# samedii/perceptor

Measured on AMD Instinct MI355X. Metric: denoising steps/sec (UNet+CLIP-grad) at 512x512 batch 8, higher is better.
Workload: dtype bf16

## Files before the change

perceptor_amd/csrc/gemm_wd.hip:

```cpp
#include "common.h"
#include "../../include/perceptor_hip.h"

namespace {

template <typename T, int MB, bool TWO = false, int NWV = 8, bool CONV = false>
__global__ __launch_bounds__(NWV * 64, 2) void gemm_wd_kernel(const pmi_igemm_args a) {
  constexpr int TM = 16 * MB, BN = NWV * 32, BK = 128, NT = NWV * 64;
  constexpr int ROW = 2 * BK + 32;
  constexpr int TILE = TM * ROW;
  constexpr int NPI = (TM * 16 + NT - 1) / NT;
  constexpr int HIMG = TM * (BN * 2 + 16);
  __shared__ __attribute__((aligned(16))) char smem[2 * TILE > 2 * HIMG ? 2 * TILE : 2 * HIMG];

  const int tid = threadIdx.x, lane = tid & 63;
  const int wid = __builtin_amdgcn_readfirstlane(tid >> 6);
#ifdef PMI_STAMPS
#define GSTAMP(k) do { if (tid == 0 && a.reserved == 77 && a.splitk <= 1) ((long long*)a.ws)[(int64_t)blockIdx.x * 8 + (k)] = (long long)wall_clock64(); } while (0)
#else
#define GSTAMP(k) do {} while (0)
#endif
  GSTAMP(0);
  const int tiles_n = (a.N + BN - 1) / BN, tiles_m = (a.M + TM - 1) / TM;
  const int logical = xcd_remap(blockIdx.x, tiles_m * tiles_n);
  const bool mfast = (int64_t)a.M <= (int64_t)a.N;
// ... 249 lines not shown
      }
      float v[4] = {c[0] * a.alpha + bv.x, c[1] * a.alpha + bv.y, c[2] * a.alpha + bv.z, c[3] * a.alpha + bv.w};
#pragma unroll
      for (int e = 0; e < 4; ++e) v[e] = act_apply(v[e], ACT);
      if (a.R) {
        if (a.res_f32) {
          const float4 rr = *(const float4*)((const float*)a.R + (int64_t)m * a.ldr + n);
          v[0] += rr.x; v[1] += rr.y; v[2] += rr.z; v[3] += rr.w;
        } else {
          const uint2 rr = *(const uint2*)((const u16*)a.R + (int64_t)m * a.ldr + n);
          v[0] += T::to_f((u16)(rr.x & 0xffff)); v[1] += T::to_f((u16)(rr.x >> 16));
          v[2] += T::to_f((u16)(rr.y & 0xffff)); v[3] += T::to_f((u16)(rr.y >> 16));
        }
      }
      if (a.out_f32) *(float4*)((float*)a.D + (int64_t)m * a.ldd + n) = make_float4(v[0], v[1], v[2], v[3]);
      else *(uint2*)((u16*)a.D + (int64_t)m * a.ldd + n) = pack4<T>(v[0], v[1], v[2], v[3]);
    }
  }
  });
  GSTAMP(3);
}

static int g_few_wgs = 128;

template <typename T>
int launch(const pmi_igemm_args& a, hipStream_t s, int mb) {
  const int tm = 16 * mb;
  const bool few = a.splitk <= 1 && (long)((a.M + 127) / 128) * ((a.N + 255) / 256) < g_few_wgs && !a.D2 && !a.aux && a.act != PMI_ACT_GEGLU;
  const bool half_tail = (a.N % 256) != 0 && (a.N % 256) <= 128 && a.N < 1024;
  if (a.N < 256 || few || half_tail) {
    const dim3 g4(((a.M + 127) / 128) * ((a.N + 127) / 128), 1, a.splitk > 1 ? a.splitk : 1);
    if (a.taps == 9) {
      if (a.A1) hipLaunchKernelGGL((gemm_wd_kernel<T, 8, true, 4, true>), g4, dim3(256), 0, s, a);
      else hipLaunchKernelGGL((gemm_wd_kernel<T, 8, false, 4, true>), g4, dim3(256), 0, s, a);
    } else if (a.A1) hipLaunchKernelGGL((gemm_wd_kernel<T, 8, true, 4>), g4, dim3(256), 0, s, a);
    else hipLaunchKernelGGL((gemm_wd_kernel<T, 8, false, 4>), g4, dim3(256), 0, s, a);
    PMI_CHECK_LAUNCH();
    return PMI_OK;
  }
  const dim3 grid(((a.M + tm - 1) / tm) * ((a.N + 255) / 256), 1, a.splitk > 1 ? a.splitk : 1);
  if (a.taps == 9) {
    if (a.A1) hipLaunchKernelGGL((gemm_wd_kernel<T, 8, true, 8, true>), grid, dim3(512), 0, s, a);
    else hipLaunchKernelGGL((gemm_wd_kernel<T, 8, false, 8, true>), grid, dim3(512), 0, s, a);
  } else if (a.A1) hipLaunchKernelGGL((gemm_wd_kernel<T, 8, true>), grid, dim3(512), 0, s, a);
  else if (mb == 9) hipLaunchKernelGGL((gemm_wd_kernel<T, 9>), grid, dim3(512), 0, s, a);
  else hipLaunchKernelGGL((gemm_wd_kernel<T, 8>), grid, dim3(512), 0, s, a);
  PMI_CHECK_LAUNCH();
  return PMI_OK;
}

}

void pmi_gemm_wd_few_wgs(int v) { g_few_wgs = v; }

int pmi_gemm_wd_tile_rows(const pmi_igemm_args* a, int splitk) {
  if (a->A1 || a->taps == 9 || a->N < 256 || ((a->N % 256) != 0 && (a->N % 256) <= 128 && a->N < 1024)) return 128;
  if (splitk <= 1 && (long)((a->M + 127) / 128) * ((a->N + 255) / 256) < g_few_wgs && !a->D2 && !a->aux && a->act != PMI_ACT_GEGLU) return 128;
  int best = 8;
  long best_cost = -1;
  for (int mb = 8; mb <= 9; ++mb) {
    const long wgs = (long)((a->M + 16 * mb - 1) / (16 * mb)) * ((a->N + 255) / 256) * (splitk > 1 ? splitk : 1);
    const long cost = ((wgs + 255) / 256) * mb;
    if (best_cost < 0 || cost < best_cost) { best_cost = cost; best = mb; }
  }
  return 16 * best;
}

int pmi_igemm_halo_allowed(void);

extern "C" int pmi_gemm_wd_eligible(const pmi_igemm_args* a) {
  if (!a->Bf || (a->taps != 1 && a->taps != 9) || a->up || a->stride != 1 || a->batch > 1) return 0;
  if (a->taps == 9) {
    if ((a->C0 % 128) || (a->A1 ? (a->C1 <= 0 || (a->C1 % 128)) : a->C1 != 0) || a->D2 || a->aux || a->act == PMI_ACT_GEGLU || a->split_in) return 0;
    if (a->H <= 0 || a->W <= 0 || a->H >= 0x4000 || a->W >= 0x4000 || a->Hin != a->H || a->Win != a->W || (a->M % (a->H * a->W))) return 0;
    if (a->K != 9 * (a->C0 + a->C1) || (int64_t)a->M * (a->lda0 > a->lda1 ? a->lda0 : a->lda1) * 2 >= ((int64_t)1 << 31)) return 0;
    if (pmi_igemm_halo_allowed() && pmi_conv3x3_halo_config(a) >= 0) return 0;
    if (a->M < 512) return 0;
  } else {
    if (a->A1 ? (a->C1 <= 0 || (a->C0 % 128) || (a->C1 % 32) || a->splitk > 1 || a->D2 || a->aux || a->act == PMI_ACT_GEGLU) : a->C1 != 0) return 0;
    if (a->K != a->C0 + a->C1) return 0;
  }
  if (a->nbias && (a->taps != 9 || a->splitk == 1)) return 0;
  if (a->res_up && (a->taps != 9 || a->splitk == 1)) return 0;
  if (a->stats || a->pro_a || a->split_out) return 0;
  if ((a->K % 32) || (a->N % 32) || a->M < 64) return 0;
  if (a->N < 256 && a->N != 128) return 0;
  if ((a->N % 256) && a->N < 1024) {
    const int tail = a->N % 256;
    if (tail < 64) return 0;
  }
  if ((a->D2 || a->aux) && (a->out_f32 || a->splitk > 1 || (a->R && a->res_f32))) return 0;
  if (a->act == PMI_ACT_GEGLU && (a->R || a->D2 || a->aux || a->out_f32 || a->splitk > 1)) return 0;
  return 1;
}

int pmi_gemm_wd_launch(const pmi_igemm_args* a, void* stream) {
  hipStream_t s = (hipStream_t)stream;
  const int mb = pmi_gemm_wd_tile_rows(a, a->splitk) / 16;
  return a->dtype == PMI_DT_BF16 ? launch<BF16>(*a, s, mb) : launch<F16>(*a, s, mb);
}
```

perceptor_amd/csrc/igemm.hip:

```cpp
#include <cstdio>
#include <cstdlib>
#include "common.h"
#include "epilogue.h"
#include "../../include/perceptor_hip.h"

namespace {

constexpr int BM = 128, BN = 128, BK = 64;
constexpr int TILE_BYTES = 128 * 128;
constexpr int STAGE_BYTES = 2 * TILE_BYTES;

__device__ __forceinline__ int lds_off(int row, int chunk) { return row * 128 + ((chunk ^ ((row >> 1) & 7)) << 4); }

template <typename T, bool CONV, bool KFAST, bool PHASED = false>
__global__ __launch_bounds__(256, 2) void igemm_kernel(const pmi_igemm_args a) {
  static_assert(!PHASED || CONV, "the phased geometry is a convolution");
  __shared__ __attribute__((aligned(16))) char smem[2 * STAGE_BYTES];

  const int tid = threadIdx.x, lane = tid & 63, wid = tid >> 6;
  const int wr = wid >> 1, wc = wid & 1;
#ifdef PMI_STAMPS
#define GSTAMP(k) do { if (tid == 0 && a.reserved == 77 && a.splitk <= 1) ((long long*)a.ws)[(int64_t)blockIdx.x * 8 + (k)] = (long long)wall_clock64(); } while (0)
#else
#define GSTAMP(k) do {} while (0)
// ... 338 lines not shown
    if (a.R) {
#pragma unroll
      for (int i = 0; i < 2; ++i)
#pragma unroll
        for (int g = 0; g < 4; ++g) {
          const int n = n0 + wc * 64 + j * 32 + 4 * lhi + 8 * g;
          rv[i][g] = make_float4(0.f, 0.f, 0.f, 0.f);
          if (mrow[i] >= a.M || n >= a.N) continue;
          if (a.res_f32) {
            rv[i][g] = *(const float4*)((const float*)a.R + offR + rrow[i] + n);
          } else if (a.split_out) {
            const int po = split_off(n, a.split_out);
            const uint2 rh = *(const uint2*)((const u16*)a.R + offR + rrow[i] + po);
            const uint2 rl = *(const uint2*)((const u16*)a.R + offR + rrow[i] + po + a.split_out);
            rv[i][g].x = __builtin_bit_cast(float, rh.x); rv[i][g].y = __builtin_bit_cast(float, rh.y);
            rv[i][g].z = __builtin_bit_cast(float, rl.x); rv[i][g].w = __builtin_bit_cast(float, rl.y);
          } else {
            const uint2 r = *(const uint2*)((const u16*)a.R + offR + rrow[i] + n);
            rv[i][g].x = __builtin_bit_cast(float, r.x); rv[i][g].y = __builtin_bit_cast(float, r.y);
          }
        }
    }
#pragma unroll
    for (int i = 0; i < 2; ++i) {
      const int m = mrow[i];
      if (m >= Mr) continue;
      const int64_t mo = orow(m);
#pragma unroll
      for (int g = 0; g < 4; ++g) {
        const int n = n0 + wc * 64 + j * 32 + 4 * lhi + 8 * g;
        if (n >= a.N) continue;
        float v[4];
#pragma unroll
        for (int e = 0; e < 4; ++e) v[e] = acc[i][j][4 * g + e] * a.alpha;
        v[0] += bv[g].x + nbv[i][g].x; v[1] += bv[g].y + nbv[i][g].y; v[2] += bv[g].z + nbv[i][g].z; v[3] += bv[g].w + nbv[i][g].w;
        if (a.act != PMI_ACT_NONE) act_apply_n<4>(v, a.act);
        if (a.R) {
          if (a.res_f32) {
            v[0] += rv[i][g].x; v[1] += rv[i][g].y; v[2] += rv[i][g].z; v[3] += rv[i][g].w;
          } else {
            const uint32_t r0 = __builtin_bit_cast(uint32_t, rv[i][g].x), r1 = __builtin_bit_cast(uint32_t, rv[i][g].y);
            v[0] += T::to_f((u16)(r0 & 0xffff)); v[1] += T::to_f((u16)(r0 >> 16));
            v[2] += T::to_f((u16)(r1 & 0xffff)); v[3] += T::to_f((u16)(r1 >> 16));
            if (a.split_out) {
              const uint32_t l0 = __builtin_bit_cast(uint32_t, rv[i][g].z), l1 = __builtin_bit_cast(uint32_t, rv[i][g].w);
              v[0] += T::to_f((u16)(l0 & 0xffff)); v[1] += T::to_f((u16)(l0 >> 16));
              v[2] += T::to_f((u16)(l1 & 0xffff)); v[3] += T::to_f((u16)(l1 >> 16));
            }
          }
        }
        if (a.split_out) {
          const int64_t o = offD + (int64_t)m * a.ldd + split_off(n, a.split_out);
          const uint2 hi = pack4<T>(v[0], v[1], v[2], v[3]);
          const float l0 = v[0] - T::to_f((u16)(hi.x & 0xffff)), l1 = v[1] - T::to_f((u16)(hi.x >> 16));
          const float l2 = v[2] - T::to_f((u16)(hi.y & 0xffff)), l3 = v[3] - T::to_f((u16)(hi.y >> 16));
          *(uint2*)((u16*)a.D + o) = hi;
          *(uint2*)((u16*)a.D + o + a.split_out) = pack4<T>(l0, l1, l2, l3);
        } else {
        const int64_t o = offD + mo * a.ldd + n;
        if (a.out_f32) *(float4*)((float*)a.D + o) = make_float4(v[0], v[1], v[2], v[3]);
        else *(uint2*)((u16*)a.D + o) = pack4<T>(v[0], v[1], v[2], v[3]);
        }
#pragma unroll
        for (int e = 0; e < 4; ++e) { ssum[4 * g + e] += v[e]; ssq[4 * g + e] += v[e] * v[e]; }
      }
    }
    if (a.stats) stats_block_to_lds(ssum, ssq, stat + wr * 2 * BN, wc * 64 + j * 32, lane);
  }
  }
  if (a.stats) {
    __syncthreads();
    const int img = m0 / a.hw, prow = (m0 - img * a.hw) / BM;
    float* o = a.stats + ((int64_t)(img * a.stats_p + prow) * a.N + n0) * 2;
    for (int c = tid; c < 2 * BN; c += 256)
      if (n0 + (c >> 1) < a.N) o[c] = stat[c] + stat[2 * BN + c];
  }
#ifdef PMI_STAMPS
  __syncthreads();
  GSTAMP(3);
#endif
}

template <typename T>
__global__ __launch_bounds__(256) void splitk_reduce_kernel(const pmi_igemm_args a) {
  const int n4 = a.N >> 2;
  const int64_t total = (int64_t)a.M * n4;
  const float* ws = (const float*)a.ws;
  for (int64_t i = (int64_t)blockIdx.x * 256 + threadIdx.x; i < total; i += (int64_t)gridDim.x * 256) {
    const int m = (int)(i / n4), n = (int)(i - (int64_t)m * n4) * 4;
    float4 s = make_float4(0.f, 0.f, 0.f, 0.f);
    for (int z = 0; z < a.splitk; ++z) {
      const float4 p = *(const float4*)(ws + ((int64_t)z * a.M + m) * a.N + n);
      s.x += p.x; s.y += p.y; s.z += p.z; s.w += p.w;
    }
    float v[4] = {s.x * a.alpha, s.y * a.alpha, s.z * a.alpha, s.w * a.alpha};
    if (a.bias) { const float4 b = *(const float4*)(a.bias + n); v[0] += b.x; v[1] += b.y; v[2] += b.z; v[3] += b.w; }
    if (a.nbias) {
      const float4 b = *(const float4*)(a.nbias + (int64_t)(m / a.hw) * (a.ldnb ? a.ldnb : a.N) + n);
      v[0] += b.x; v[1] += b.y; v[2] += b.z; v[3] += b.w;
    }
    if (a.act != PMI_ACT_NONE) act_apply_n<4>(v, a.act);
    if (a.R) {
      int64_t rrow = (int64_t)m * a.ldr;
      if (a.res_up) {
        const int hw = a.H * a.W;
        const int img = m / hw, rem = m - img * hw;
        const int y = rem / a.W, x = rem - y * a.W;
        rrow = ((int64_t)(img * (a.H >> 1) + (y >> 1)) * (a.W >> 1) + (x >> 1)) * a.ldr;
      }
      if (a.res_f32) {
        const float4 r = *(const float4*)((const float*)a.R + rrow + n);
        v[0] += r.x; v[1] += r.y; v[2] += r.z; v[3] += r.w;
      } else {
        const int po = a.split_out ? split_off(n, a.split_out) : n;
        const uint2 r = *(const uint2*)((const u16*)a.R + rrow + po);
        v[0] += T::to_f((u16)(r.x & 0xffff)); v[1] += T::to_f((u16)(r.x >> 16));
        v[2] += T::to_f((u16)(r.y & 0xffff)); v[3] += T::to_f((u16)(r.y >> 16));
        if (a.split_out) {
          const uint2 l = *(const uint2*)((const u16*)a.R + rrow + po + a.split_out);
          v[0] += T::to_f((u16)(l.x & 0xffff)); v[1] += T::to_f((u16)(l.x >> 16));
          v[2] += T::to_f((u16)(l.y & 0xffff)); v[3] += T::to_f((u16)(l.y >> 16));
        }
      }
    }
    if (a.split_out) {
      const int64_t o = (int64_t)m * a.ldd + split_off(n, a.split_out);
      const uint2 hi = pack4<T>(v[0], v[1], v[2], v[3]);
      const float l0 = v[0] - T::to_f((u16)(hi.x & 0xffff)), l1 = v[1] - T::to_f((u16)(hi.x >> 16));
      const float l2 = v[2] - T::to_f((u16)(hi.y & 0xffff)), l3 = v[3] - T::to_f((u16)(hi.y >> 16));
      *(uint2*)((u16*)a.D + o) = hi;
      *(uint2*)((u16*)a.D + o + a.split_out) = pack4<T>(l0, l1, l2, l3);
      continue;
    }
    const int64_t o = (int64_t)m * a.ldd + n;
    if (a.out_f32) *(float4*)((float*)a.D + o) = make_float4(v[0], v[1], v[2], v[3]);
    else *(uint2*)((u16*)a.D + o) = pack4<T>(v[0], v[1], v[2], v[3]);
  }
}

template <typename T>
int launch(const pmi_igemm_args& a, hipStream_t s) {
  const bool phased = a.up == 2;
  const int tiles = (((phased ? a.M / 4 : a.M) + BM - 1) / BM) * ((a.N + BN - 1) / BN);
  const dim3 grid(tiles, phased ? 4 : 1, a.batch > 1 ? a.batch : (a.splitk > 1 ? a.splitk : 1)), block(256);
  const bool conv = a.taps != 1 || a.up || a.stride == 2;
  const int Cin = a.C0 + a.C1;
  const bool kfast = (Cin % BK == 0) && (a.C0 % BK == 0);
  if (phased) {
    if (kfast) hipLaunchKernelGGL((igemm_kernel<T, true, true, true>), grid, block, 0, s, a);
    else hipLaunchKernelGGL((igemm_kernel<T, true, false, true>), grid, block, 0, s, a);
  } else if (conv) {
    if (kfast) hipLaunchKernelGGL((igemm_kernel<T, true, true>), grid, block, 0, s, a);
    else hipLaunchKernelGGL((igemm_kernel<T, true, false>), grid, block, 0, s, a);
  } else {
    if (kfast) hipLaunchKernelGGL((igemm_kernel<T, false, true>), grid, block, 0, s, a);
    else hipLaunchKernelGGL((igemm_kernel<T, false, false>), grid, block, 0, s, a);
  }
  PMI_CHECK_LAUNCH();
  if (a.splitk > 1) {
    const int64_t work = (int64_t)a.M * (a.N / 4);
    const int blocks = (int)((work + 255) / 256 > 4096 ? 4096 : (work + 255) / 256);
    hipLaunchKernelGGL(splitk_reduce_kernel<T>, dim3(blocks), dim3(256), 0, s, a);
    PMI_CHECK_LAUNCH();
  }
  return PMI_OK;
}

}

extern "C" int pmi_conv3x3_halo_config(const pmi_igemm_args* a);
int pmi_conv3x3_halo_launch(const pmi_igemm_args* a, int cfg, void* stream);
int pmi_conv3x3_wd_launch(const pmi_igemm_args* a, int cfg, void* stream);
extern "C" int pmi_gemm_wd_eligible(const pmi_igemm_args* a);
int pmi_gemm_wd_tile_rows(const pmi_igemm_args* a, int splitk);
int pmi_gemm_wd_launch(const pmi_igemm_args* a, void* stream);
void pmi_conv3x3_allow_wd(int v);
void pmi_conv3x3_wd_mf16(int v);
void pmi_conv3x3_wd128(int v);
void pmi_conv3x3_force_config(int cfg);
void pmi_conv3x3_prefer_256(int v);
static int g_allow_halo = 1;
static int g_wd_max_split = 8;
int pmi_conv3x3_wd_splitk(const pmi_igemm_args* a, int cfg);
extern "C" int pmi_igemm_splitk(const pmi_igemm_args* a) {
  if (a->batch > 1 || (a->N & 3) || a->up == 2) return 1;
  if (g_allow_halo) {
    const int halo = pmi_conv3x3_halo_config(a);
    if (halo >= 0) return pmi_conv3x3_wd_splitk(a, halo);
  }
  if (a->act == PMI_ACT_GEGLU) return 1;
  if (a->A1 && a->taps == 1 && pmi_gemm_wd_eligible(a)) return 1;
  if (pmi_gemm_wd_eligible(a)) {
    const int nch = (a->K + 127) / 128;
    int best = 1;
    long best_cost = -1;
    for (int s = 1; s <= g_wd_max_split && nch / s >= 4; s *= 2) {
      const int rows = pmi_gemm_wd_tile_rows(a, s);
      const long wgs = (long)((a->M + rows - 1) / rows) * (a->N < 256 ? 1 : (a->N + 255) / 256) * s;
      const long cost = ((wgs + 255) / 256) * rows * (nch / s + 6) + (s > 1 ? 8L * 144 : 0);
      if (best_cost < 0 || cost < best_cost) { best_cost = cost; best = s; }
    }
    return best;
  }
  const int tiles = ((a->M + BM - 1) / BM) * ((a->N + BN - 1) / BN);
  const int nk = (a->K + BK - 1) / BK;
  if (tiles >= 384 || nk < 16) return 1;
  int s = 512 / tiles;
  if (s > nk / 8) s = nk / 8;
  if (s > 16) s = 16;
  return s < 2 ? 1 : s;
}

int pmi_igemm_halo_allowed(void) { return g_allow_halo; }

extern "C" int pmi_igemm_stats_rows(const pmi_igemm_args* a) {
  if (a->batch > 1 || a->splitk > 1 || a->up == 2) return 0;
  const int halo = g_allow_halo ? pmi_conv3x3_halo_config(a) : -1;
  if (a->split_out) return halo >= 6 ? (a->H / 8) * (a->W / 32) : 0;
  if (halo == 3) return 0;
  if (halo >= 0) return (a->H / (halo == 1 ? 16 : 8)) * (a->W / 32);
  if (a->hw > 0 && (a->hw % BM) == 0 && (a->M % a->hw) == 0) return a->hw / BM;
  return 0;
}

void pmi_attn_flash_qt(int v);
void pmi_attn_flash_kv_chunks(int v);
void pmi_conv3x3_wd_splitk_enable(int v);
void pmi_gemm_wd_few_wgs(int v);
void pmi_conv3x3_wd_smallc(int v);

extern "C" int pmi_set_option(int key, int value) {
  if (key == 0) { const int old = g_allow_halo; g_allow_halo = value; return old; }
  if (key == 1) { pmi_conv3x3_force_config(value); return 0; }
  if (key == 2) { pmi_conv3x3_prefer_256(value); return 0; }
  if (key == 6) { pmi_conv3x3_allow_wd(value); return 0; }
  if (key == 7) { pmi_conv3x3_wd_mf16(value); return 0; }
  if (key == 8) { pmi_conv3x3_wd128(value); return 0; }
  if (key == 9) { pmi_attn_flash_qt(value); return 0; }
  if (key == 10) { pmi_conv3x3_wd_splitk_enable(value); return 0; }
  if (key == 11) { g_wd_max_split = value; return 0; }
  if (key == 12) { pmi_gemm_wd_few_wgs(value); return 0; }
  if (key == 13) { pmi_conv3x3_wd_smallc(value); return 0; }
  if (key == 14) { pmi_attn_flash_kv_chunks(value); return 0; }
  return PMI_ERR_ARG;
}

static int bad_arg(int line) {
  if (getenv("PMI_DEBUG")) fprintf(stderr, "pmi_igemm: argument check at igemm.hip:%d failed\n", line);
  return PMI_ERR_ARG;
}

extern "C" int pmi_igemm(const pmi_igemm_args* a, pmi_stream_t stream) {
  if (!a || !a->A0 || !a->B || !a->D) return bad_arg(__LINE__);
  if (a->M <= 0 || a->N <= 0 || a->K <= 0) return bad_arg(__LINE__);
  if ((a->K & 7) || (a->C0 & 7) || (a->C1 & 7)) return bad_arg(__LINE__);
  if ((a->N & 3) && (a->bias || a->nbias || a->R || a->ldd < ((a->N + 3) & ~3))) return bad_arg(__LINE__);
  if ((a->lda0 & 7) || (a->ldb & 7) || (a->ldd & 3)) return bad_arg(__LINE__);
  if (a->C1 > 0 && (!a->A1 || (a->lda1 & 7))) return bad_arg(__LINE__);
  if (a->taps != 1 && a->taps != 9 && a->taps != 16) return bad_arg(__LINE__);
  if (a->taps == 16 && (a->stride != 2 || a->up || a->res_up || a->Hin != 2 * a->H || a->Win != 2 * a->W)) return bad_arg(__LINE__);
  if (a->stride != 1 && a->stride != 2) return bad_arg(__LINE__);
  if (a->up == 2 && (a->taps != 9 || a->stride != 2 || a->res_up || a->A1 || a->C1 || a->R || a->nbias || a->stats || a->splitk > 1 || a->batch > 1 ||
                     a->split_out || a->split_in || a->pro_a || a->D2 || a->aux || a->dtype == PMI_DT_F16X2 || (a->M & 3))) return bad_arg(__LINE__);
  if (a->K != a->taps * (a->C0 + a->C1)) return bad_arg(__LINE__);
  if (a->R && (a->ldr & 3)) return bad_arg(__LINE__);
  if (a->split_out && ((a->split_out & 7) || a->split_out > 32 || a->out_f32 || (a->N % a->split_out) || a->batch > 1)) return bad_arg(__LINE__);
  if ((unsigned)a->split_in > 2u) return bad_arg(__LINE__);
  if (a->split_in == 2 && !a->split_out) return bad_arg(__LINE__);
  if (a->nbias && a->hw <= 0) return bad_arg(__LINE__);
  const bool conv = a->taps != 1 || a->up || a->stride == 2;
  if (a->res_up && ((a->H & 1) || (a->W & 1))) return bad_arg(__LINE__);
  if ((conv || a->res_up) && (a->H <= 0 || a->W <= 0 || a->Hin <= 0 || a->Win <= 0 || a->M % (a->H * a->W))) return bad_arg(__LINE__);
  if (a->up && (a->H != 2 * a->Hin || a->W != 2 * a->Win)) return bad_arg(__LINE__);
  if (a->batch > 1 && a->batch_inner <= 0) return bad_arg(__LINE__);
  const int halo = g_allow_halo ? pmi_conv3x3_halo_config(a) : -1;
  if (a->pro_a && (!a->pro_b || halo < 0)) return PMI_ERR_ARG;
  if ((a->split_in == 2 || ((a->split_in || a->split_out) && a->pro_a) || (a->split_out && a->R && a->res_f32)) && halo < 6) return bad_arg(__LINE__);
  if (a->stats && a->stats_p != pmi_igemm_stats_rows(a)) return PMI_ERR_ARG;
  if (a->splitk > 1 && (!a->ws || a->batch > 1 || (halo >= 0 && a->splitk != pmi_conv3x3_wd_splitk(a, halo)) || (a->N & 3) || a->stats)) return PMI_ERR_ARG;
  if (a->act == PMI_ACT_GEGLU && !pmi_gemm_wd_eligible(a)) return bad_arg(__LINE__);
  if ((a->D2 || a->aux) && !pmi_gemm_wd_eligible(a)) return bad_arg(__LINE__);
  if (pmi_gemm_wd_eligible(a) && !((a->nbias || a->res_up) && a->splitk <= 1)) {
    const int rc = pmi_gemm_wd_launch(a, stream);
    if (rc != PMI_OK || a->splitk <= 1 || a->reserved3 == 1) return rc;
    hipStream_t s = (hipStream_t)stream;
    const int64_t work = (int64_t)a->M * (a->N / 4);
    const int blocks = (int)((work + 255) / 256 > 4096 ? 4096 : (work + 255) / 256);
    if (a->dtype == PMI_DT_BF16) hipLaunchKernelGGL(splitk_reduce_kernel<BF16>, dim3(blocks), dim3(256), 0, s, *a);
    else hipLaunchKernelGGL(splitk_reduce_kernel<F16>, dim3(blocks), dim3(256), 0, s, *a);
    PMI_CHECK_LAUNCH();
    return PMI_OK;
  }
  if (halo >= 4) {
    const int rc = pmi_conv3x3_wd_launch(a, halo, stream);
    if (rc != PMI_OK || a->splitk <= 1) return rc;
    hipStream_t s = (hipStream_t)stream;
    const int64_t work = (int64_t)a->M * (a->N / 4);
    const int blocks = (int)((work + 255) / 256 > 4096 ? 4096 : (work + 255) / 256);
    if (a->dtype == PMI_DT_BF16) hipLaunchKernelGGL(splitk_reduce_kernel<BF16>, dim3(blocks), dim3(256), 0, s, *a);
    else hipLaunchKernelGGL(splitk_reduce_kernel<F16>, dim3(blocks), dim3(256), 0, s, *a);
    PMI_CHECK_LAUNCH();
    return PMI_OK;
  }
  if (halo >= 0) return pmi_conv3x3_halo_launch(a, halo, stream);
  hipStream_t s = (hipStream_t)stream;
  return a->dtype == PMI_DT_BF16 ? launch<BF16>(*a, s) : launch<F16>(*a, s);
}

extern "C" int pmi_abi_version(void) { return 1; }
```

perceptor_amd/engine/ops.py:

```python
from __future__ import annotations

import math
import os
import ctypes as C
from typing import Optional

import torch

from .. import _hip
from .._hip import ACT_GEGLU, ACT_NONE, DT_F16X2, IgemmArgs, call, ptr


HALO_ENABLED = True
SPLITK_ENABLED = True
WD_ENABLED = True
GEMM_WD_ENABLED = True
GEMM_WD_CONV = os.environ.get("PMI_GEMM_WD_CONV", "1") != "0"
FLASH_ENABLED = True


def set_halo(enabled: bool) -> None:
    global HALO_ENABLED
    HALO_ENABLED = bool(enabled)
    _hip.lib().pmi_set_option(0, int(enabled))
# ... 251 lines not shown
    a.pro_a, a.pro_b, a.pro_act = ptr(ca), ptr(cb), pact
    out = _empty((n, h, w, 2 * lin.n_p), torch.float16, x.device)
    a.D, a.ldd = ptr(out), out.stride(-2)
    rows = _hip.lib().pmi_igemm_stats_rows(C.byref(a))
    if rows > 0:
        st = _empty((n, rows, lin.n_p, 2), torch.float32, x.device)
        a.stats, a.stats_p = ptr(st), rows
        out._pmi_stats = (st, rows)
    if DEBUG_WS is not None:
        a.ws = ptr(DEBUG_WS)
        a.reserved = 77
    if KERNEL_EVENTS is not None:
        e0, e1 = torch.cuda.Event(enable_timing=True), torch.cuda.Event(enable_timing=True)
        e0.record()
        call("pmi_igemm", C.byref(a))
        e1.record()
        nbytes = (x.numel() + (x1.numel() if x1 is not None else 0)) * 2 + lin.w.numel() * 2 + out.numel() * 2 + (residual.numel() * 2 if residual is not None else 0)
        KERNEL_EVENTS.append((e0, e1, 2.0 * m * lin.cout * lin.cin * 9, float(nbytes), f"{h}x{w} {c0}+{c1}->{lin.cout} cfg{cfg} mixed-{operand}"))
        return out
    call("pmi_igemm", C.byref(a))
    return out


def igemm(a0: torch.Tensor, lin: PackedLinear, *, a1: Optional[torch.Tensor] = None, residual: Optional[torch.Tensor] = None,
          act: int = ACT_NONE, up: bool = False, stride: int = 1, res_up: bool = False, nbias: Optional[torch.Tensor] = None,
          out_f32: bool = False, out: Optional[torch.Tensor] = None, alpha: float = 1.0, prologue=None,
          want_stats: bool = False, hw: Optional[int] = None, pre_out: Optional[torch.Tensor] = None,
          act_grad_of: Optional[torch.Tensor] = None, act_grad: int = ACT_NONE, defer_reduce: bool = False,
          split_out: bool = False) -> torch.Tensor:
    dt = lin.dt
    conv = a0.ndim == 4
    if lin.concat_inputs and a1 is not None and prologue is None:
        a0, a1 = torch.cat([a0, a1], dim=-1), None
    c0 = a0.shape[-1]
    c1 = a1.shape[-1] if a1 is not None else 0
    assert (c0 + c1) * (2 if lin.self_concat else 1) == lin.cin_p, (c0, c1, lin.cin_p)
    a = IgemmArgs()
    if conv:
        n, hin, win, _ = a0.shape
        hv, wv = (hin * 2, win * 2) if up else (hin, win)
        h, w = hv // stride, wv // stride
        m = n * h * w
        a.H, a.W, a.Hin, a.Win = h, w, hin, win
        a.hw = h * w
        oshape = (n, h, w, lin.n_p)
    else:
        assert lin.taps == 1 and not up and stride == 1
        m = a0.shape[0]
        a.hw = hw or 1
        oshape = (m, lin.n_p // 2 if act == ACT_GEGLU else lin.n_p)
    if lin.split:
        a.split_in = 1
    if (lin.split and not out_f32) or split_out:
        a.split_out = split_group(lin.n_p)
        oshape = oshape[:-1] + (2 * lin.n_p,)
    if out is None:
        out = _empty(oshape, torch.float32 if out_f32 else _hip.TORCH_DTYPE[dt], a0.device)
    a.A0, a.A1, a.B = ptr(a0), ptr(a1), ptr(lin.w)
    a.bias, a.nbias, a.R, a.D = ptr(lin.b), ptr(nbias), ptr(residual), ptr(out)
    a.M, a.N, a.K = m, lin.n_p, lin.K
    a.C0, a.C1 = c0, c1
    a.lda0, a.lda1 = a0.stride(-2), (a1.stride(-2) if a1 is not None else 0)
    a.ldb, a.ldd = lin.K, out.stride(-2)
    a.ldr = residual.stride(-2) if residual is not None else 0
    a.taps, a.stride, a.up, a.res_up, a.act = lin.taps, stride, int(up), int(res_up), act
    a.out_f32 = int(out.dtype == torch.float32)
    a.res_f32 = int(residual is not None and residual.dtype == torch.float32)
    a.alpha = alpha
    a.ldnb = nbias.stride(0) if nbias is not None else 0
    a.batch, a.batch_inner = 1, 1
    a.dtype = dt
    if conv and lin.taps == 9 and stride == 1 and HALO_ENABLED and WD_ENABLED and lin.n_p % 32 == 0 and ((lin.n_p >= 128 and lin.cin_p % 64 == 0) or (lin.cin_p <= 32 and a1 is None)):
        a.Bf = 1
        a.pro_a = 1 if (prologue is not None and not lin.split) else None
        cfg = _hip.lib().pmi_conv3x3_halo_config(C.byref(a))
        a.pro_a = None
        a.Bf = ptr(lin.frag16(64)) if cfg == 6 else ptr(lin.frag16(32)) if cfg == 7 else ptr(lin.frag(64)) if cfg == 4 else ptr(lin.frag_c8()) if cfg == 8 else None
    if pre_out is not None or act_grad_of is not None:
        a.D2, a.aux, a.aux_act = ptr(pre_out), ptr(act_grad_of), act_grad
    wd_ok = GEMM_WD_ENABLED and lin.taps == 1 and (not lin.split or out_f32) and not up and stride == 1 and lin.n_p % 32 == 0 and lin.K % 32 == 0 \
        and nbias is None and prologue is None
    if wd_ok and want_stats:
        wd_ok = SPLITK_ENABLED and _hip.lib().pmi_igemm_splitk(C.byref(a)) > 1
    if wd_ok:
        a.Bf = 1
        a.Bf = ptr(lin.frag_gemm()) if _hip.lib().pmi_gemm_wd_eligible(C.byref(a)) else None
        if a.Bf:
            want_stats = False
    if prologue is not None:
        ca, cb, pact = prologue
        if HALO_ENABLED and not lin.split and _hip.lib().pmi_conv3x3_halo_config(C.byref(a)) >= 0:
            a.pro_a, a.pro_b, a.pro_act = ptr(ca), ptr(cb), pact
        else:
            if lin.split and a1 is not None and (c0 // 2) % 32 + (c1 // 2) % 32:
                raise ValueError(f"precise two-source prologue: sources of {c0 // 2} + {c1 // 2} channels are not both multiples of 32")
            n_, h_, w_, _ = a0.shape
            y = _empty((n_, h_, w_, c0 + c1), a0.dtype, a0.device)
            lc0, lc = (c0 // 2, (c0 + c1) // 2) if lin.split else (c0, c0 + c1)
            call("pmi_gn_apply", ptr(a0), ptr(a1), lc0, ptr(ca), ptr(cb), None, ptr(y), n_, h_, w_, lc, pact, 0, dt)
            a.A0, a.A1, a.C0, a.C1, a.lda0, a.lda1 = ptr(y), None, c0 + c1, 0, c0 + c1, 0
            a0 = y
    if lin.self_concat:
        assert a.A1 is None
        a.A1, a.C1, a.lda1 = a.A0, a.C0, a.lda0
    conv_gemm = False
    if conv and lin.taps == 9 and stride == 1 and not up and GEMM_WD_ENABLED and GEMM_WD_CONV and not lin.split and not a.Bf \
            and not a.pro_a and lin.n_p % 32 == 0 and c0 % 128 == 0 and c1 % 128 == 0:
        a.Bf = 1
        a.Bf = ptr(lin.frag_gemm()) if _hip.lib().pmi_gemm_wd_eligible(C.byref(a)) else None
        conv_gemm = bool(a.Bf)
    if SPLITK_ENABLED:
        sk = _hip.lib().pmi_igemm_splitk(C.byref(a))
        if sk > 1:
            ws = _empty((sk, m, lin.n_p), torch.float32, a0.device)
            a.ws, a.splitk = ptr(ws), sk
            if defer_reduce and a.Bf and not conv and _hip.lib().pmi_gemm_wd_eligible(C.byref(a)):
                a.reserved3 = 1
                call("pmi_igemm", C.byref(a))
                return ("slabs", ws, sk)
    if conv_gemm and (nbias is not None or res_up) and a.splitk <= 1:
        a.Bf = None
    if want_stats:
        rows = _hip.lib().pmi_igemm_stats_rows(C.byref(a))
        if rows > 0:
            st = _empty((m // a.hw, rows, lin.n_p, 2), torch.float32, a0.device)
            a.stats, a.stats_p = ptr(st), rows
            out._pmi_stats = (st, rows)
    if DEBUG_WS is not None and a.splitk <= 1:
        a.ws = ptr(DEBUG_WS)
        a.reserved = 77
    if KERNEL_EVENTS is not None and lin.taps == 9 and HALO_ENABLED and _hip.lib().pmi_conv3x3_halo_config(C.byref(a)) >= 0:
        e0, e1 = torch.cuda.Event(enable_timing=True), torch.cuda.Event(enable_timing=True)
        e0.record()
        call("pmi_igemm", C.byref(a))
        e1.record()
        nbytes = (a0.numel() + (a1.numel() if a1 is not None else 0)) * 2 + lin.w.numel() * 2 + out.numel() * out.element_size()
        if residual is not None:
            nbytes += (residual.numel() if not res_up else residual.numel()) * residual.element_size()
        desc = f"{a.H}x{a.W} {c0}+{c1}->{lin.cout} cfg{_hip.lib().pmi_conv3x3_halo_config(C.byref(a))}" \
               f"{' pro' if prologue is not None else ''}{' res' if residual is not None else ''}{' up' if up else ''}{' stats' if want_stats else ''}"
        KERNEL_EVENTS.append((e0, e1, 2.0 * m * lin.cout * lin.cin * lin.taps, float(nbytes), desc))
        return out
    if GEMM_TRACE is not None:
        kind = "conv" if conv and (lin.taps == 9 or up or stride == 2) else "gemm"
        desc = f"{kind} M={m} N={lin.n_p} K={lin.K} taps={lin.taps}{' up' if up else ''}{' s2' if stride == 2 else ''} splitk={a.splitk}" \
               f" halo={_hip.lib().pmi_conv3x3_halo_config(C.byref(a)) if HALO_ENABLED else -1} wd={int(bool(a.Bf) and bool(_hip.lib().pmi_gemm_wd_eligible(C.byref(a))))}" \
               f"{' res' if residual is not None else ''}{' f32out' if a.out_f32 else ''}{' nbias' if nbias is not None else ''}{' stats' if a.stats else ''}" \
               f"{' split_in' if a.split_in else ''}{' split_out' if a.split_out else ''}{' self_concat' if lin.self_concat else ''}"
        e0, e1 = torch.cuda.Event(enable_timing=True), torch.cuda.Event(enable_timing=True)
        e0.record()
        call("pmi_igemm", C.byref(a))
        e1.record()
        GEMM_TRACE.append((desc, 2.0 * m * lin.n_p * lin.K, e0, e1))
        return out
    call("pmi_igemm", C.byref(a))
    return out


def downsample_adjoint_args(g: torch.Tensor, lin: PackedLinear, out: torch.Tensor) -> IgemmArgs:
    n, h, w, c = g.shape
    a = IgemmArgs()
    a.A0, a.B, a.D = ptr(g), ptr(lin.w), ptr(out)
    a.M, a.N, a.K = 4 * n * h * w, lin.n_p, lin.K
    a.C0, a.lda0, a.ldb, a.ldd = c, g.stride(-2), lin.K, out.stride(-2)
    a.H, a.W, a.Hin, a.Win, a.hw = 2 * h, 2 * w, h, w, 4 * h * w
    a.taps, a.stride, a.up = 9, 2, 2
    a.out_f32 = int(out.dtype == torch.float32)
    a.alpha = 1.0
    a.batch, a.batch_inner = 1, 1
    a.dtype = lin.dt
    return a


def downsample_adjoint(g: torch.Tensor, lin: PackedLinear, *, out_f32: bool = False, out: Optional[torch.Tensor] = None) -> torch.Tensor:
    n, h, w, c = g.shape
    assert lin.taps == 9 and not lin.split and c == lin.cin_p, (lin.taps, c, lin.cin_p)
    if out is None:
        out = _empty((n, 2 * h, 2 * w, lin.n_p), torch.float32 if out_f32 else _hip.TORCH_DTYPE[lin.dt], g.device)
    call("pmi_igemm", C.byref(downsample_adjoint_args(g, lin, out)))
    return out


def geglu_linear(x: torch.Tensor, lin: PackedLinear) -> torch.Tensor:
    dt = lin.dt
    a = IgemmArgs()
    a.taps, a.stride, a.M, a.N, a.K, a.C0, a.batch, a.Bf, a.act = 1, 1, x.shape[0], lin.n_p, lin.K, lin.K, 1, 1, ACT_GEGLU
    if GEMM_WD_ENABLED and not lin.split and lin.n_p % 32 == 0 and lin.K % 32 == 0 and _hip.lib().pmi_gemm_wd_eligible(C.byref(a)):
        return igemm(x, lin, act=ACT_GEGLU)
    f = igemm(x, lin)
    out = _empty((x.shape[0], lin.n_p // 2), f.dtype, f.device)
    call("pmi_geglu", ptr(f), ptr(out), x.shape[0], lin.n_p // 2, 1, dt)
    return out


def interleave_geglu(weight: torch.Tensor, bias: Optional[torch.Tensor]):
    f = weight.shape[0] // 2
    assert f % 16 == 0
    idx = torch.arange(f).view(-1, 16)
    perm = torch.cat([idx, idx + f], dim=1).flatten()
    return weight[perm].contiguous(), (bias[perm].contiguous() if bias is not None else None)


def fused_mlp_epilogues(lin: PackedLinear, m: int) -> bool:
    if not (GEMM_WD_ENABLED and lin.taps == 1 and not lin.split and lin.n_p % 256 == 0 and lin.K % 128 == 0 and m >= 64):
# ... 535 lines not shown
```

Before: 25.37.

## Fuse GroupNorm statistics into split-K reduction kernel

Adds a split-K reduce variant that, besides summing the fp32 slabs and applying the epilogue, accumulates per-channel sum and sum-of-squares over pixel tiles and writes partial stats rows. Split-K GEMMs and convs that feed a GroupNorm can now produce stats inline instead of needing a separate statistics pass. This also lets wide GEMMs keep split-K when stats are requested. The stats reduce uses a 3D grid with shared-memory partials, which may give a less efficient reduce layout than the grid-stride kernel.

```diff
diff --git a/perceptor_amd/csrc/gemm_wd.hip b/perceptor_amd/csrc/gemm_wd.hip
--- a/perceptor_amd/csrc/gemm_wd.hip
+++ b/perceptor_amd/csrc/gemm_wd.hip
@@ -355,7 +355,7 @@
   }
   if (a->nbias && (a->taps != 9 || a->splitk == 1)) return 0;
   if (a->res_up && (a->taps != 9 || a->splitk == 1)) return 0;
-  if (a->stats || a->pro_a || a->split_out) return 0;
+  if ((a->stats && a->splitk <= 1) || a->pro_a || a->split_out) return 0;
   if ((a->K % 32) || (a->N % 32) || a->M < 64) return 0;
   if (a->N < 256 && a->N != 128) return 0;
   if ((a->N % 256) && a->N < 1024) {
diff --git a/perceptor_amd/csrc/igemm.hip b/perceptor_amd/csrc/igemm.hip
--- a/perceptor_amd/csrc/igemm.hip
+++ b/perceptor_amd/csrc/igemm.hip
@@ -444,47 +444,53 @@
 }
 
 template <typename T>
+__device__ __forceinline__ void splitk_reduce_elem(const pmi_igemm_args& a, int m, int n, float* v) {
+  const float* ws = (const float*)a.ws;
+  float4 s = make_float4(0.f, 0.f, 0.f, 0.f);
+  for (int z = 0; z < a.splitk; ++z) {
+    const float4 p = *(const float4*)(ws + ((int64_t)z * a.M + m) * a.N + n);
+    s.x += p.x; s.y += p.y; s.z += p.z; s.w += p.w;
+  }
+  v[0] = s.x * a.alpha; v[1] = s.y * a.alpha; v[2] = s.z * a.alpha; v[3] = s.w * a.alpha;
+  if (a.bias) { const float4 b = *(const float4*)(a.bias + n); v[0] += b.x; v[1] += b.y; v[2] += b.z; v[3] += b.w; }
+  if (a.nbias) {
+    const float4 b = *(const float4*)(a.nbias + (int64_t)(m / a.hw) * (a.ldnb ? a.ldnb : a.N) + n);
+    v[0] += b.x; v[1] += b.y; v[2] += b.z; v[3] += b.w;
+  }
+  if (a.act != PMI_ACT_NONE) act_apply_n<4>(v, a.act);
+  if (a.R) {
+    int64_t rrow = (int64_t)m * a.ldr;
+    if (a.res_up) {
+      const int hw = a.H * a.W;
+      const int img = m / hw, rem = m - img * hw;
+      const int y = rem / a.W, x = rem - y * a.W;
+      rrow = ((int64_t)(img * (a.H >> 1) + (y >> 1)) * (a.W >> 1) + (x >> 1)) * a.ldr;
+    }
+    if (a.res_f32) {
+      const float4 r = *(const float4*)((const float*)a.R + rrow + n);
+      v[0] += r.x; v[1] += r.y; v[2] += r.z; v[3] += r.w;
+    } else {
+      const int po = a.split_out ? split_off(n, a.split_out) : n;
+      const uint2 r = *(const uint2*)((const u16*)a.R + rrow + po);
+      v[0] += T::to_f((u16)(r.x & 0xffff)); v[1] += T::to_f((u16)(r.x >> 16));
+      v[2] += T::to_f((u16)(r.y & 0xffff)); v[3] += T::to_f((u16)(r.y >> 16));
+      if (a.split_out) {
+        const uint2 l = *(const uint2*)((const u16*)a.R + rrow + po + a.split_out);
+        v[0] += T::to_f((u16)(l.x & 0xffff)); v[1] += T::to_f((u16)(l.x >> 16));
+        v[2] += T::to_f((u16)(l.y & 0xffff)); v[3] += T::to_f((u16)(l.y >> 16));
+      }
+    }
+  }
+}
+
+template <typename T>
 __global__ __launch_bounds__(256) void splitk_reduce_kernel(const pmi_igemm_args a) {
   const int n4 = a.N >> 2;
   const int64_t total = (int64_t)a.M * n4;
-  const float* ws = (const float*)a.ws;
   for (int64_t i = (int64_t)blockIdx.x * 256 + threadIdx.x; i < total; i += (int64_t)gridDim.x * 256) {
     const int m = (int)(i / n4), n = (int)(i - (int64_t)m * n4) * 4;
-    float4 s = make_float4(0.f, 0.f, 0.f, 0.f);
-    for (int z = 0; z < a.splitk; ++z) {
-      const float4 p = *(const float4*)(ws + ((int64_t)z * a.M + m) * a.N + n);
-      s.x += p.x; s.y += p.y; s.z += p.z; s.w += p.w;
-    }
-    float v[4] = {s.x * a.alpha, s.y * a.alpha, s.z * a.alpha, s.w * a.alpha};
-    if (a.bias) { const float4 b = *(const float4*)(a.bias + n); v[0] += b.x; v[1] += b.y; v[2] += b.z; v[3] += b.w; }
-    if (a.nbias) {
-      const float4 b = *(const float4*)(a.nbias + (int64_t)(m / a.hw) * (a.ldnb ? a.ldnb : a.N) + n);
-      v[0] += b.x; v[1] += b.y; v[2] += b.z; v[3] += b.w;
-    }
-    if (a.act != PMI_ACT_NONE) act_apply_n<4>(v, a.act);
-    if (a.R) {
-      int64_t rrow = (int64_t)m * a.ldr;
-      if (a.res_up) {
-        const int hw = a.H * a.W;
-        const int img = m / hw, rem = m - img * hw;
-        const int y = rem / a.W, x = rem - y * a.W;
-        rrow = ((int64_t)(img * (a.H >> 1) + (y >> 1)) * (a.W >> 1) + (x >> 1)) * a.ldr;
-      }
-      if (a.res_f32) {
-        const float4 r = *(const float4*)((const float*)a.R + rrow + n);
-        v[0] += r.x; v[1] += r.y; v[2] += r.z; v[3] += r.w;
-      } else {
-        const int po = a.split_out ? split_off(n, a.split_out) : n;
-        const uint2 r = *(const uint2*)((const u16*)a.R + rrow + po);
-        v[0] += T::to_f((u16)(r.x & 0xffff)); v[1] += T::to_f((u16)(r.x >> 16));
-        v[2] += T::to_f((u16)(r.y & 0xffff)); v[3] += T::to_f((u16)(r.y >> 16));
-        if (a.split_out) {
-          const uint2 l = *(const uint2*)((const u16*)a.R + rrow + po + a.split_out);
-          v[0] += T::to_f((u16)(l.x & 0xffff)); v[1] += T::to_f((u16)(l.x >> 16));
-          v[2] += T::to_f((u16)(l.y & 0xffff)); v[3] += T::to_f((u16)(l.y >> 16));
-        }
-      }
-    }
+    float v[4];
+    splitk_reduce_elem<T>(a, m, n, v);
     if (a.split_out) {
       const int64_t o = (int64_t)m * a.ldd + split_off(n, a.split_out);
       const uint2 hi = pack4<T>(v[0], v[1], v[2], v[3]);
@@ -498,6 +504,61 @@
     if (a.out_f32) *(float4*)((float*)a.D + o) = make_float4(v[0], v[1], v[2], v[3]);
     else *(uint2*)((u16*)a.D + o) = pack4<T>(v[0], v[1], v[2], v[3]);
   }
+}
+
+constexpr int RS_PIX = 32, RS_CH = 64;
+template <typename T>
+__global__ __launch_bounds__(256) void splitk_reduce_stats_kernel(const pmi_igemm_args a) {
+  __shared__ float part[16][RS_CH][2];
+  const int tid = threadIdx.x, cq = tid & 15, pl = tid >> 4;
+  const int img = blockIdx.z, p0 = blockIdx.y * RS_PIX;
+  const int n = blockIdx.x * RS_CH + 4 * cq;
+  float cs[4] = {0.f, 0.f, 0.f, 0.f}, cq2[4] = {0.f, 0.f, 0.f, 0.f};
+  if (n < a.N) {
+#pragma unroll
+    for (int j = 0; j < RS_PIX / 16; ++j) {
+      const int p = p0 + pl + 16 * j;
+      if (p >= a.hw) break;
+      const int m = img * a.hw + p;
+      float v[4];
+      splitk_reduce_elem<T>(a, m, n, v);
+      const uint2 pk = pack4<T>(v[0], v[1], v[2], v[3]);
+      *(uint2*)((u16*)a.D + (int64_t)m * a.ldd + n) = pk;
+      const float f[4] = {T::to_f((u16)(pk.x & 0xffff)), T::to_f((u16)(pk.x >> 16)), T::to_f((u16)(pk.y & 0xffff)), T::to_f((u16)(pk.y >> 16))};
+#pragma unroll
+      for (int e = 0; e < 4; ++e) { cs[e] += f[e]; cq2[e] += f[e] * f[e]; }
+    }
+  }
+#pragma unroll
+  for (int e = 0; e < 4; ++e) { part[pl][4 * cq + e][0] = cs[e]; part[pl][4 * cq + e][1] = cq2[e]; }
+  __syncthreads();
+  if (tid < 2 * RS_CH) {
+    const int c = tid >> 1, k = tid & 1;
+    if (blockIdx.x * RS_CH + c < a.N) {
+      float t = 0.f;
+#pragma unroll
+      for (int l = 0; l < 16; ++l) t += part[l][c][k];
+      a.stats[(((int64_t)img * a.stats_p + blockIdx.y) * a.N + blockIdx.x * RS_CH) * 2 + tid] = t;
+    }
+  }
+}
+
+static int g_reduce_stats = 1;
+inline int reduce_stats_rows(const pmi_igemm_args& a) {
+  if (!g_reduce_stats || a.out_f32 || a.split_out || a.hw <= 0 || (a.M % a.hw) || (a.N & 3)) return 0;
+  return (a.hw + RS_PIX - 1) / RS_PIX;
+}
+
+template <typename T>
+void launch_reduce(const pmi_igemm_args& a, hipStream_t s) {
+  if (a.stats) {
+    const dim3 grid((a.N + RS_CH - 1) / RS_CH, a.stats_p, a.M / a.hw);
+    hipLaunchKernelGGL(splitk_reduce_stats_kernel<T>, grid, dim3(256), 0, s, a);
+    return;
+  }
+  const int64_t work = (int64_t)a.M * (a.N / 4);
+  const int blocks = (int)((work + 255) / 256 > 4096 ? 4096 : (work + 255) / 256);
+  hipLaunchKernelGGL(splitk_reduce_kernel<T>, dim3(blocks), dim3(256), 0, s, a);
 }
 
 template <typename T>
@@ -520,9 +581,7 @@
   }
   PMI_CHECK_LAUNCH();
   if (a.splitk > 1) {
-    const int64_t work = (int64_t)a.M * (a.N / 4);
-    const int blocks = (int)((work + 255) / 256 > 4096 ? 4096 : (work + 255) / 256);
-    hipLaunchKernelGGL(splitk_reduce_kernel<T>, dim3(blocks), dim3(256), 0, s, a);
+    launch_reduce<T>(a, s);
     PMI_CHECK_LAUNCH();
   }
   return PMI_OK;
@@ -576,7 +635,8 @@
 int pmi_igemm_halo_allowed(void) { return g_allow_halo; }
 
 extern "C" int pmi_igemm_stats_rows(const pmi_igemm_args* a) {
-  if (a->batch > 1 || a->splitk > 1 || a->up == 2) return 0;
+  if (a->batch > 1 || a->up == 2) return 0;
+  if (a->splitk > 1) return reduce_stats_rows(*a);
   const int halo = g_allow_halo ? pmi_conv3x3_halo_config(a) : -1;
   if (a->split_out) return halo >= 6 ? (a->H / 8) * (a->W / 32) : 0;
   if (halo == 3) return 0;
@@ -604,6 +664,7 @@
   if (key == 12) { pmi_gemm_wd_few_wgs(value); return 0; }
   if (key == 13) { pmi_conv3x3_wd_smallc(value); return 0; }
   if (key == 14) { pmi_attn_flash_kv_chunks(value); return 0; }
+  if (key == 15) { g_reduce_stats = value; return 0; }
   return PMI_ERR_ARG;
 }
 
@@ -639,17 +700,15 @@
   if (a->pro_a && (!a->pro_b || halo < 0)) return PMI_ERR_ARG;
   if ((a->split_in == 2 || ((a->split_in || a->split_out) && a->pro_a) || (a->split_out && a->R && a->res_f32)) && halo < 6) return bad_arg(__LINE__);
   if (a->stats && a->stats_p != pmi_igemm_stats_rows(a)) return PMI_ERR_ARG;
-  if (a->splitk > 1 && (!a->ws || a->batch > 1 || (halo >= 0 && a->splitk != pmi_conv3x3_wd_splitk(a, halo)) || (a->N & 3) || a->stats)) return PMI_ERR_ARG;
+  if (a->splitk > 1 && (!a->ws || a->batch > 1 || (halo >= 0 && a->splitk != pmi_conv3x3_wd_splitk(a, halo)) || (a->N & 3))) return PMI_ERR_ARG;
   if (a->act == PMI_ACT_GEGLU && !pmi_gemm_wd_eligible(a)) return bad_arg(__LINE__);
   if ((a->D2 || a->aux) && !pmi_gemm_wd_eligible(a)) return bad_arg(__LINE__);
   if (pmi_gemm_wd_eligible(a) && !((a->nbias || a->res_up) && a->splitk <= 1)) {
     const int rc = pmi_gemm_wd_launch(a, stream);
     if (rc != PMI_OK || a->splitk <= 1 || a->reserved3 == 1) return rc;
     hipStream_t s = (hipStream_t)stream;
-    const int64_t work = (int64_t)a->M * (a->N / 4);
-    const int blocks = (int)((work + 255) / 256 > 4096 ? 4096 : (work + 255) / 256);
-    if (a->dtype == PMI_DT_BF16) hipLaunchKernelGGL(splitk_reduce_kernel<BF16>, dim3(blocks), dim3(256), 0, s, *a);
-    else hipLaunchKernelGGL(splitk_reduce_kernel<F16>, dim3(blocks), dim3(256), 0, s, *a);
+    if (a->dtype == PMI_DT_BF16) launch_reduce<BF16>(*a, s);
+    else launch_reduce<F16>(*a, s);
     PMI_CHECK_LAUNCH();
     return PMI_OK;
   }
@@ -657,10 +716,8 @@
     const int rc = pmi_conv3x3_wd_launch(a, halo, stream);
     if (rc != PMI_OK || a->splitk <= 1) return rc;
     hipStream_t s = (hipStream_t)stream;
-    const int64_t work = (int64_t)a->M * (a->N / 4);
-    const int blocks = (int)((work + 255) / 256 > 4096 ? 4096 : (work + 255) / 256);
-    if (a->dtype == PMI_DT_BF16) hipLaunchKernelGGL(splitk_reduce_kernel<BF16>, dim3(blocks), dim3(256), 0, s, *a);
-    else hipLaunchKernelGGL(splitk_reduce_kernel<F16>, dim3(blocks), dim3(256), 0, s, *a);
+    if (a->dtype == PMI_DT_BF16) launch_reduce<BF16>(*a, s);
+    else launch_reduce<F16>(*a, s);
     PMI_CHECK_LAUNCH();
     return PMI_OK;
   }
diff --git a/perceptor_amd/engine/ops.py b/perceptor_amd/engine/ops.py
--- a/perceptor_amd/engine/ops.py
+++ b/perceptor_amd/engine/ops.py
@@ -357,11 +357,11 @@
         and nbias is None and prologue is None
     if wd_ok and want_stats:
         wd_ok = SPLITK_ENABLED and _hip.lib().pmi_igemm_splitk(C.byref(a)) > 1
+    wd_gemm = False
     if wd_ok:
         a.Bf = 1
         a.Bf = ptr(lin.frag_gemm()) if _hip.lib().pmi_gemm_wd_eligible(C.byref(a)) else None
-        if a.Bf:
-            want_stats = False
+        wd_gemm = bool(a.Bf)
     if prologue is not None:
         ca, cb, pact = prologue
         if HALO_ENABLED and not lin.split and _hip.lib().pmi_conv3x3_halo_config(C.byref(a)) >= 0:
@@ -395,6 +395,8 @@
                 return ("slabs", ws, sk)
     if conv_gemm and (nbias is not None or res_up) and a.splitk <= 1:
         a.Bf = None
+    if wd_gemm and a.splitk <= 1:
+        want_stats = False
     if want_stats:
         rows = _hip.lib().pmi_igemm_stats_rows(C.byref(a))
         if rows > 0:
```

Result: no change. 25.52, median of 6 (+0.6%).
